# fnzhan/EMLight

Hardware: AMD Instinct MI355X
Metric: training images/sec (regression step: DenseNet-BC fwd + Sinkhorn loss + bwd + Adam) (higher is better)
Workload: dtype f32; 1 GPU; RegressionNetwork train step, BASELINE configs[1]; per_gpu_batch=64, global_batch=64, anchors=128, parallelism=single

## Files before the change

### emlight_amd/RegressionNetwork/dense_engine_bwd.py

```python
import ctypes
import os

import torch

from .. import _lib
from .._knobs import knob_choice, knob_flag


def _r16(v):
    return (v + 15) // 16 * 16


def _side_stream(dev, prio):
    if prio <= 0:
        return torch.cuda.Stream(device=dev, priority=prio)
    hip = ctypes.CDLL("libamdhip64.so")
    h = ctypes.c_void_p()
    with torch.cuda.device(dev):
        rc = hip.hipStreamCreateWithPriority(ctypes.byref(h), ctypes.c_uint(1), ctypes.c_int(prio))
    if rc != 0:
        raise RuntimeError("hipStreamCreateWithPriority failed (%d)" % rc)
    return torch.cuda.ExternalStream(h.value, device=dev)


# ... 15 lines not shown
class _BwdBuffers:
    def gf12(self, r):
        if self.GF12[r] is None:
            self.GF12[r] = self._gf12_new()
        return self.GF12[r]

    def __init__(self, enc, ws, dev):
        f32 = dict(dtype=torch.float32, device=dev)
        self.G = [torch.zeros(blk["P"], blk["ld"], **f32) for blk in ws.blocks]
        self.GF = torch.zeros(ws.F.shape[0], ws.F.shape[1], **f32)
        maxP = ws.blocks[0]["P"]
        self.DZ = torch.empty(2, maxP, 48, **f32)
        self.ring = max(1, int(os.environ.get("EML_WGRAD_RING", 4))) if enc.overlap_wgrad(dev) else 1
        self.GF12 = [None] * self.ring
        self._gf12_new = lambda: torch.empty(maxP, 12, **f32)
        self.N12 = torch.empty(maxP, 12, **f32)
        self.TOP = torch.empty(2 * maxP * 12, **f32) if knob_flag("EML_DGRAD_TOP", True) else None
        kp, ko, g = enc.kp_max, max(enc.ko_max, 48), enc.grid_max
        self.Wd = [[torch.empty(lay["Kp"] * 48, **f32) for lay in blk["layers"]] for blk in ws.blocks]
        self.WdT = [torch.empty(blk["trans"]["Kp"] * blk["trans"]["Ko"], **f32) for blk in ws.blocks]
        self.permutes = None
        self.coef = torch.zeros(8, max(kp, ko), **f32)
        self.part2 = torch.zeros(2, g * kp * 2, dtype=torch.float64, device=dev)
        self.partW = torch.empty(g * max(kp * 48, 2 * 27 * 256, 4 * 1024), **f32)
        i32 = dict(dtype=torch.int32, device=dev)
        self.cond = [[torch.zeros(lay["Kp"], **i32) for lay in blk["layers"]] for blk in ws.blocks]
        self.condT = [torch.zeros(blk["trans"]["Kp"], **i32) for blk in ws.blocks]
        self.any_ill = torch.zeros(1, **i32)
        self.dg_grid = 128
        self.dg_scratch = torch.empty(self.dg_grid * kp, dtype=torch.float64, device=dev)
        self.side = None
        if enc.overlap_wgrad(dev):
            m = int(os.environ.get("EML_CU_SPLIT", 0))
            self.main_masked = None
            if m > 1:
                n_cu = torch.cuda.get_device_properties(dev).multi_processor_count
                self.side = _masked_stream(dev, n_cu, lambda i: i % m == m - 1)
                self.main_masked = _masked_stream(dev, n_cu, lambda i: i % m != m - 1)
            else:
                self.side = _side_stream(dev, int(os.environ.get("EML_SIDE_PRIO", 0)))
            self.partW3 = [torch.empty(g * 2 * 27 * 256, **f32) for _ in range(self.ring)]
            self.ev_ready = [torch.cuda.Event() for _ in range(self.ring)]
            self.ev_done = [None] * self.ring


def run_backward(enc, ws, x, gpooled, need_x=False, need_params=None):
    if getattr(ws, "bwd", None) is None:
        ws.bwd = _BwdBuffers(enc, ws, x.device)
    masked = getattr(ws.bwd, "main_masked", None)
    if masked is None:
        return _run_backward(enc, ws, x, gpooled, need_x, need_params)
    cur = torch.cuda.current_stream(x.device)
    masked.wait_stream(cur)
# ... 85 lines not shown
                                                    blk["P"], st), "eml_dense_grad_materialize_f32")

    cf, k = enc.trans_cout[-1], enc.avgpool
    ldF = ws.F.shape[1]
    _lib.check(L.eml_dense_head_pool_bwd_f32(p(gpooled), p(ws.F), ldF, cf, B, ws.hf, ws.wf, k, p(bw.GF), ldF, st),
               "eml_dense_head_pool_bwd_f32")
    dY, ld_dy = bw.GF, ldF
    nb = len(ws.blocks)
    for bi in reversed(range(nb)):
        blk, tr = ws.blocks[bi], ws.blocks[bi]["trans"]
        mod = getattr(f, "denseblock%d" % (bi + 1))
        T, LN = getattr(f, "transition%d" % (bi + 1)), getattr(f, "last_norm%d" % (bi + 1))
        P, Hb, Wb, ld, ctot = blk["P"], blk["H"], blk["W"], blk["ld"], blk["Ctot"]
        cout, Ko, kpt = tr["Cout"], tr["Ko"], tr["Kp"]
        Pn = B * (Hb // 2) * (Wb // 2)
        Gbuf = bw.G[bi]
        gl0 = sum(enc.block_layers[:bi])
        top2 = bw.TOP[:2 * P * 12].view(2, P, 12) if bw.TOP is not None else None
        _lib.check(L.eml_dense_bn_bwd_stats_f32(p(dY), ld_dy, p(tr["T"]), Ko, None, 0, 0, cout, Pn, p(tr["tmean"]),
                                                p(tr["tistd"]), p(part), Gb, st), "eml_dense_bn_bwd_stats_f32")
        finalize(Gb, 2 * cout, Pn, LN, tr["tmean"], tr["tistd"], cout, Ko, coef=0)
        _lib.check(L.eml_dense_conv1x1_bwd_weight_f32(
            p(tr["A"]), kpt, Pn, Hb // 2, Wb // 2, 0, kpt, ctot, p(tr["one"]), p(tr["zero"]), p(dY), ld_dy, p(tr["T"]),
            Ko, p(cA), p(cB), p(cC), cout, p(bw.partW), gr(T.conv.weight), G, None, None, 0, None, 0, None, None, st),
            "eml_dense_conv1x1_bwd_weight_f32")
        _lib.check(L.eml_dense_conv1x1_bwd_data_f32(
            p(dY), ld_dy, p(tr["T"]), Ko, p(cA), p(cB), p(cC), Ko, p(bw.WdT[bi]), None, ld, p(tr["scale"]),
            p(tr["shift"]), None, None, Pn, Hb, Wb, 1, kpt, p(Gbuf), ld, 0, p(part), G, p(tr["mask16"]), st),
            "eml_dense_conv1x1_bwd_data_f32")
        finalize(G, 2 * kpt, P, T.norm, blk["mean"], blk["istd"], ctot, kpt, coef=None, s_acc=False, conv=T.conv,
                 cond=bw.condT[bi])
        dgamma_direct(blk, ld, P, Hb, Wb, 1, dY, ld_dy, tr["T"], Ko, coefs[0], cout, T.conv, ctot, tr["scale"], tr["shift"],
                      bw.condT[bi], T.norm)
        def conv2_backward(l, slot, n12=False, narrow_lo=None, top=False):
            lay = blk["layers"][l]
            Lm = getattr(mod, "denselayer%d" % (l + 1))
            cin, kp, z, dz = lay["Cin"], lay["Kp"], blk["Z"][l], bw.DZ[slot]
            gsrc = (p(bw.N12), 12, 0) if n12 else (p(top2[1]), 12, 0) if top else (p(Gbuf), ld, cin)
            r = ring[0] = (ring[0] + 1) % bw.ring
            if bw.side is not None and bw.ev_done[r] is not None:
                main.wait_event(bw.ev_done[r])
            fold = (bw.side is None and c3_fold
                    and L.eml_dense_conv3x3_bwd_fused_supported(gsrc[1], gsrc[2], ld, cin) == 1)
            q = ws.drop_plan[bi][l] if ws.drop_plan is not None else 0.0
            drop = (ws.drop_key, gl0 + l, q) if q > 0 else ()
            if fold:
                fn = "eml_dense_conv3x3_bwd_fused_drop_f32" if drop else "eml_dense_conv3x3_bwd_fused_f32"
# ... 40 lines not shown
                    parr([bw.part2[s_] for s_ in slots]), (ctypes.c_int * len(layers))(*[y["Kp"] for y in lays]),
                    P, k_hi, p(Gbuf), ld, Gd, parr([y["mask"] for y in lays]), p(top2), st),
                    "eml_dense_conv1x1_bwd_data_multi_top_f32")
                return
            _lib.check(L.eml_dense_conv1x1_bwd_data_multi_f32(
                len(layers), parr([bw.DZ[s_] for s_ in slots]), None, None, None, None,
                parr([bw.Wd[bi][l_] for l_ in layers]),
                parr([y["scale1"] for y in lays]), parr([y["shift1"] for y in lays]),
                parr([bw.part2[s_] for s_ in slots]), (ctypes.c_int * len(layers))(*[y["Kp"] for y in lays]),
                None, ld, None, None, P, k_lo, k_hi, p(Gbuf), ld, Gd,
                parr([y["mask"] for y in lays]), st),
                "eml_dense_conv1x1_bwd_data_multi_f32")

        def bn1_finalize(l, Lm, slot, c_lo, c_hi, rows=None):
            lay = blk["layers"][l]
            finalize(Gd if rows is None else rows, 2 * lay["Kp"], P, Lm.norm1, blk["mean"], blk["istd"], lay["Cin"], lay["Kp"], coef=None,
                     s_acc=True, src=bw.part2[slot], c_lo=c_lo, c_hi=c_hi, conv=Lm.conv1, cond=bw.cond[bi][l])

        def bn1_direct(l, Lm, slot):
            lay = blk["layers"][l]
            dgamma_direct(blk, ld, P, Hb, Wb, 0, bw.DZ[slot], 48, None, 0, None, 48, Lm.conv1, lay["Cin"], lay["scale1"],
                          lay["shift1"], bw.cond[bi][l], Lm.norm1)

        l = len(blk["layers"]) - 1
        have_top = False
        while l >= 0:
            if l >= 1:
                la, lb = l, l - 1
                cin_a, cin_b = blk["layers"][la]["Cin"], blk["layers"][lb]["Cin"]
                Lma = conv2_backward(la, 0, narrow_lo=cin_b, top=have_top)
                bn1_finalize(la, Lma, 0, cin_b, cin_a, rows=Gw)
                Lmb = conv2_backward(lb, 1, n12=True)
                to_top = (top2 is not None and lb >= 2 and blk["layers"][la]["mask"] is not None and bw.side is None
                          and cin_b >= 24 and cin_b % 4 == 0)
                dgrad([la, lb], [0, 1], 0, cin_b, top=to_top)
                have_top = to_top
                bn1_finalize(la, Lma, 0, 0, cin_b)
                bn1_finalize(lb, Lmb, 1, 0, blk["layers"][lb]["Kp"])
                bn1_direct(la, Lma, 0)
                bn1_direct(lb, Lmb, 1)
                l -= 2
            else:
                Lm0 = conv2_backward(l, 0)
                dgrad([l], [0], 0, blk["layers"][l]["Cin"])
                bn1_finalize(l, Lm0, 0, 0, blk["layers"][l]["Kp"])
                bn1_direct(l, Lm0, 0)
                l -= 1
        c0b = blk["C0"]
        norm0_fused = bi == 0 and knob_flag("EML_NORM0_FUSED", True) and c0b % 4 == 0 and c0b <= 32
        if not norm0_fused:
            materialize(Gbuf, blk, 0, c0b)
        dY, ld_dy = Gbuf, ld
    b0 = ws.blocks[0]
    c0 = enc.c_init
    if norm0_fused:
        _lib.check(L.eml_dense_norm0_bwd_stats_f32(p(dY), ld_dy, p(ws.Y0), c0, p(ws.scale0), p(ws.shift0), p(sB), p(sC), c0,
                                                   b0["P"], p(ws.mean0), p(ws.istd0), p(part), Gb, st),
                   "eml_dense_norm0_bwd_stats_f32")
    else:
        _lib.check(L.eml_dense_bn_bwd_stats_f32(p(dY), ld_dy, p(ws.Y0), c0, p(b0["X"]), b0["ld"], 1, c0, b0["P"],
                                                p(ws.mean0), p(ws.istd0), p(part), Gb, st), "eml_dense_bn_bwd_stats_f32")
    finalize(Gb, 2 * c0, b0["P"], f.norm0, ws.mean0, ws.istd0, c0, _r16(c0), coef=0)
    if norm0_fused:
# ... 18 lines not shown
```

### emlight_amd/_lib.py

```python
import ctypes
import os
import threading

_HERE = os.path.dirname(os.path.abspath(__file__))
LIB_PATH = os.environ.get("EML_LIB_PATH") or os.path.join(_HERE, "libemlight_hip.so")

_f32p = ctypes.c_void_p
_i32p = ctypes.c_void_p
_f64p = ctypes.c_void_p
_stream = ctypes.c_void_p
_int = ctypes.c_int
_u64 = ctypes.c_ulonglong

ABI_VERSION = 31

SIGNATURES = {
    "eml_abi_version": (_int, []),
    "eml_last_error": (ctypes.c_char_p, []),
    "eml_sg_rasterise_f32": (_int, [_f32p, _f32p, _f32p, _f32p, _int, _int, _int, _int, _stream]),
    "eml_sg_rasterise_ex_f32": (_int, [_f32p, _f32p, _f32p, _f32p, _int, _int, _int, _int, _int, ctypes.c_void_p, _stream]),
    "eml_sg_rasterise_bwd_colors_f32": (_int, [_f32p, _f32p, _f32p, _f32p, _int, _int, _int, _int, _stream]),
    "eml_emd_anchor_cost_f32": (_int, [_f32p, _f32p, _int, _stream]),
    "eml_sinkhorn_schedule_f32": (_int, [_f32p, _f32p, ctypes.c_long, ctypes.c_double, ctypes.c_double, _int,
                                         ctypes.c_double, _f32p, _f32p, _i32p, _f32p, _stream]),
# ... 135 lines not shown
    "eml_dense_dropout_mask_u16": (_int, [_u64, _int, ctypes.c_double, ctypes.c_long, ctypes.c_void_p, _stream]),
    "eml_dense_pool_act_f32": (_int, [_f32p, _int, _int, _int, _int, _int, _f32p, _f32p, _f32p, _int, ctypes.c_void_p,
                                      _stream]),
    "eml_dense_head_pool_fwd_f32": (_int, [_f32p, _int, _int, _int, _int, _int, _int, _f32p, _stream]),
    "eml_dense_conv3x3_bwd_data_f32": (_int, [_f32p, _int, _int, _f32p, _f32p, _f32p, _f32p, _f32p, _int, _int, _int,
                                              _f32p, _int, _f32p, _int, _int, _f32p, _f32p, _f32p, _stream]),
    "eml_dense_conv3x3_bwd_fused_supported": (_int, [_int, _int, _int, _int]),
    "eml_dense_conv3x3_bwd_fused_f32": (_int, [_f32p, _int, _int, _f32p, _f32p, _f32p, _f32p, _f32p, _int, _int, _int, _f64p, _int,
                                               _f32p, _int, _int, _f32p, _f32p, _f32p, _f32p, _f32p, _f32p, _f32p, _stream]),
    "eml_dense_conv3x3_bwd_data_drop_f32": (_int, [_f32p, _int, _int, _f32p, _f32p, _f32p, _f32p, _f32p, _int, _int, _int,
                                                   _f32p, _int, _f32p, _int, _int, _f32p, _f32p, _f32p, _u64, _int,
                                                   ctypes.c_double, _stream]),
    "eml_dense_conv3x3_bwd_fused_drop_f32": (_int, [_f32p, _int, _int, _f32p, _f32p, _f32p, _f32p, _f32p, _int, _int, _int,
                                                    _f64p, _int, _f32p, _int, _int, _f32p, _f32p, _f32p, _f32p, _f32p, _f32p,
                                                    _f32p, _u64, _int, ctypes.c_double, _stream]),
    "eml_dense_conv3x3_bwd_weight_f32": (_int, [_f32p, _int, _int, _f32p, _f32p, _f32p, _int, _int, _int, _f32p,
                                                _f32p, _int, _stream]),
    "eml_dense_bn_bwd_finalize_f32": (_int, [_f32p, _int, _int, ctypes.c_double, _f32p, _f32p, _f32p, _int, _int,
                                             _int, _f32p, _f32p, _f32p, _f32p, _f32p, _f32p, _f32p, _int, _int, _int,
                                             _f32p, _f32p, _f32p, _int, _i32p, _i32p, _stream]),
    "eml_dense_bn_dgamma_direct_f32": (_int, [_f32p, _int, ctypes.c_long, _int, _int, _int, _f32p, _int, _f32p, _int,
                                              _f32p, _f32p, _f32p, _int, _f32p, _int, _f32p, _f32p, _f32p, _f32p, _i32p,
                                              _f32p, _f32p, _int, _stream]),
    "eml_dense_conv1x1_bwd_weight_f32": (_int, [_f32p, _int, ctypes.c_long, _int, _int, _int, _int, _int, _f32p,
                                                _f32p, _f32p, _int, _f32p, _int, _f32p, _f32p, _f32p, _int, _f32p,
                                                _f32p, _int, _f32p, _f32p, _int, _f32p, _int, _f32p, _f32p, _stream]),
    "eml_dense_conv1x1_bwd_narrow_f32": (_int, [_f32p, _f32p, _int, _int, _f32p, _int, _f32p, _f32p, _f32p, _f32p,
                                                ctypes.c_long, _f32p, _int, _f32p, _f32p, _int, _int, _stream]),
    "eml_dense_permute_w1_bwd_f32": (_int, [_f32p, _int, _int, _int, _int, _f32p, _stream]),
    "eml_dense_conv1x1_bwd_data_f32": (_int, [_f32p, _int, _f32p, _int, _f32p, _f32p, _f32p, _int, _f32p, _f32p,
                                              _int, _f32p, _f32p, _f32p, _f32p, ctypes.c_long, _int, _int, _int,
                                              _int, _f32p, _int, _int, _f32p, _int, ctypes.c_void_p, _stream]),
    "eml_dense_conv1x1_bwd_data_multi_f32": (_int, [_int] + [ctypes.c_void_p] * 10 + [_f32p, _int, _f32p, _f32p,
                                                    ctypes.c_long, _int, _int, _f32p, _int, _int, ctypes.c_void_p,
                                                    _stream]),
    "eml_dense_conv1x1_bwd_data_multi_top_f32": (_int, [ctypes.c_void_p] * 6 + [ctypes.c_long, _int, _f32p, _int, _int,
                                                        ctypes.c_void_p, _f32p, _stream]),
    "eml_dense_grad_materialize_f32": (_int, [_f32p, _int, _f32p, _int, _f32p, _f32p, _int, _int, ctypes.c_long,
                                              _stream]),
    "eml_dense_bn_bwd_stats_f32": (_int, [_f32p, _int, _f32p, _int, _f32p, _int, _int, _int, ctypes.c_long, _f32p,
                                          _f32p, _f32p, _int, _stream]),
    "eml_dense_norm0_bwd_stats_f32": (_int, [_f32p, _int, _f32p, _int, _f32p, _f32p, _f32p, _f32p, _int, ctypes.c_long, _f32p, _f32p,
                                             ctypes.c_void_p, _int, _stream]),
    "eml_dense_conv0_bwd_weight_fused_f32": (_int, [_f32p, _f32p, _int, _f32p, _int, _f32p, _f32p, _f32p, _f32p, _f32p, _f32p, _f32p,
                                                    _int, _int, _int, _f32p, _f32p, _int, _stream]),
    "eml_dense_conv0_bwd_weight_f32": (_int, [_f32p, _f32p, _int, _f32p, _int, _f32p, _int, _f32p, _f32p, _f32p,
# ... 79 lines not shown
```

### emlight_amd/csrc/dense_bwd.hip

```cpp
#include "eml_common.h"
#include "eml_dropout.h"

#include <cstdint>
#include <cstdlib>
#include <type_traits>

namespace {

using f32x4 = __attribute__((ext_vector_type(4))) float;

__device__ __forceinline__ f32x4 mfma16(float a, float b, f32x4 c) {
  return __builtin_amdgcn_mfma_f32_16x16x4f32(a, b, c, 0, 0, 0);
}
__device__ __forceinline__ float f4c(const float4& v, int t) { return t == 0 ? v.x : t == 1 ? v.y : t == 2 ? v.z : v.w; }
__device__ __forceinline__ double shfl_xor_d(double v, int m) { return __shfl_xor(v, m, 64); }

constexpr int kTH = 8, kTW = 32, kHH = kTH + 2, kHW = kTW + 2;

constexpr int kPSG = 14;
constexpr int kBD = 512;
constexpr int kGRows = 2;
constexpr int kGPass = kHH / kGRows;

template <bool FUSE, bool WIDE, int TH, bool DROP = false>
// ... 1415 lines not shown
#pragma unroll
      for (int g = 0; g < 4; ++g) {
        const int ch = GW * cg + VEC * (4 * kk + g) + t;
        if (cg < ngroups && ch < Kp) {
#pragma unroll
          for (int n = 0; n < 3; ++n) out[(size_t)ch * 48 + 16 * n + r] = acc[i][t][n][g];
        }
      }
  }
  if constexpr (NARROW) {
    __syncthreads();
    double* red = reinterpret_cast<double*>(&dz_l[0][0]);
#pragma unroll
    for (int g = 0; g < 4; ++g) {
#pragma unroll
      for (int o = 1; o < 16; o <<= 1) ns1[g] += shfl_xor_d(ns1[g], o);
      if (r == 0 && kk < 3) red[wave * 12 + 4 * kk + g] = ns1[g];
    }
    __syncthreads();
    if (tid < 12) {
      double* dst = na.partials + ((size_t)blockIdx.x * Kp + na.k_lo + tid) * 2;
      dst[0] = (red[tid] + red[12 + tid]) + (red[24 + tid] + red[36 + tid]);
      dst[1] = 0.0;
    }
  }
}

template <bool POOL, bool RES , int NCH = 4>
__global__ __launch_bounds__(256) void conv1x1_bwd_data_kernel(
    const float* __restrict__ DY, int ld_dy, const float* __restrict__ Zr, int ld_z, const float* __restrict__ cA,
    const float* __restrict__ cB, const float* __restrict__ cC, int Ko, const float* __restrict__ Wd,
    const float* __restrict__ X, int ldx, const float* __restrict__ scale1, const float* __restrict__ shift1,
    const float* __restrict__ mean, const float* __restrict__ istd, int P, int Hin, int Win, int Kp,
    float* __restrict__ Gd, int ldg, int accumulate, double* __restrict__ partials ) {
  extern __shared__ __attribute__((aligned(16))) float smem[];
  double* sacc = reinterpret_cast<double*>(smem);
  const int tid = threadIdx.x, lane = tid & 63, wave = tid >> 6;
  const int r = lane & 15, kk = lane >> 4;
  for (int e = tid; e < 4 * Kp * 2; e += 256) sacc[e] = 0.0;
  __syncthreads();
  double* my = sacc + (size_t)wave * Kp * 2;
  const int nnt = Kp >> 4, njo = Ko >> 4;
  const int ntiles = (P + 255) >> 8;
  const int Wo = Win >> 1, Ho = Hin >> 1;

  for (int tile = blockIdx.x; tile < ntiles; tile += gridDim.x) {
// ... 1118 lines not shown
}

__global__ __launch_bounds__(256) void head_pool_bwd_kernel(const float* __restrict__ gp, const float* __restrict__ F,
                                                            int ldf, int C, int B, int H, int W, int k,
                                                            float* __restrict__ dF, int ldd) {
  const int Ho = H / k, Wo = W / k;
  const size_t total = (size_t)B * H * W * C;
  const float inv = 1.0f / (float)(k * k);
  for (size_t e = (size_t)blockIdx.x * 256 + threadIdx.x; e < total; e += (size_t)gridDim.x * 256) {
    const int c = (int)(e % C);
    const size_t p = e / C;
    const int xx = (int)(p % W);
    const size_t rest = p / W;
    const int yy = (int)(rest % H), b = (int)(rest / H);
    const int oy = yy / k, ox = xx / k;
    float v = 0.f;
    if (oy < Ho && ox < Wo && F[p * ldf + c] > 0.f) v = gp[(((size_t)b * C + c) * Ho + oy) * Wo + ox] * inv;
    dF[p * ldd + c] = v;
  }
}

}

__global__ __launch_bounds__(256) void bn_dgamma_direct_partial_kernel(
    const float* __restrict__ X, int ldx, long P, int Hin, int Win, int pool, const float* __restrict__ DY, int ld_dy,
    const float* __restrict__ Zr, int ld_z, const float* __restrict__ cA, const float* __restrict__ cB,
    const float* __restrict__ cC, int Cout, const float* __restrict__ W, int Cin, const float* __restrict__ scale1,
    const float* __restrict__ shift1, const float* __restrict__ mean, const float* __restrict__ istd,
    const int* __restrict__ cond, double* __restrict__ partial) {
  __shared__ int list[384];
  __shared__ int cnt;
  __shared__ float wcol[192], co[3][192];
  __shared__ double red[4];
  const int tid = threadIdx.x;
  if (tid == 0) cnt = 0;
  __syncthreads();
  for (int c = tid; c < Cin; c += 256)
    if (cond[c]) list[atomicAdd(&cnt, 1)] = c;
  __syncthreads();
  const int n = cnt;
  if (n == 0) return;
  for (int o = tid; o < Cout; o += 256) {
    co[0][o] = Zr ? cA[o] : 1.f;
    co[1][o] = Zr ? cB[o] : 0.f;
    co[2][o] = Zr ? cC[o] : 0.f;
  }
  const long per = (P + gridDim.x - 1) / gridDim.x, p_lo = (long)blockIdx.x * per, p_hi = min(P, p_lo + per);
  const int Ho = Hin >> 1, Wo = Win >> 1;
  for (int li = 0; li < n; ++li) {
    const int c = list[li];
    __syncthreads();
    for (int o = tid; o < Cout; o += 256) wcol[o] = W[(size_t)o * Cin + c];
    __syncthreads();
    const float s1 = scale1[c], t1 = shift1[c];
    const double mu = mean[c], is = istd[c];
    double acc = 0.0;
    for (long p = p_lo + tid; p < p_hi; p += 256) {
      const float x = X[(size_t)p * ldx + c];
      if (fmaf(x, s1, t1) > 0.f) {
        long pp = p;
        if (pool) {
          const long b = p / ((long)Hin * Win), rem = p - b * (long)Hin * Win;
          const int y = (int)(rem / Win), xx = (int)(rem - (long)y * Win);
          pp = (b * Ho + (y >> 1)) * Wo + (xx >> 1);
        }
        const float* dy = DY + (size_t)pp * ld_dy;
        const float* zr = Zr ? Zr + (size_t)pp * ld_z : dy;
        double d = 0.0;
        for (int o = 0; o < Cout; ++o) d += (double)wcol[o] * (double)fmaf(co[0][o], dy[o], fmaf(co[1][o], zr[o], co[2][o]));
        if (pool) d *= 0.25;
        acc += d * (((double)x - mu) * is);
      }
    }
#pragma unroll
    for (int o = 32; o > 0; o >>= 1) acc += shfl_xor_d(acc, o);
    if ((tid & 63) == 0) red[tid >> 6] = acc;
    __syncthreads();
    if (tid == 0) partial[(size_t)blockIdx.x * Cin + c] = (red[0] + red[1]) + (red[2] + red[3]);
  }
}

__global__ __launch_bounds__(256) void bn_dgamma_direct_reduce_kernel(const double* __restrict__ partial, int R, int Cin,
                                                                      const int* __restrict__ cond,
                                                                      float* __restrict__ dgamma) {
  const int c = blockIdx.x * 256 + threadIdx.x;
  if (c >= Cin || !cond[c]) return;
  double s = 0.0;
  for (int g = 0; g < R; ++g) s += partial[(size_t)g * Cin + c];
  dgamma[c] = (float)s;
}

extern "C" int eml_dense_conv3x3_bwd_data_f32(const float* G, int ldg, int c0, const float* W2, const float* Z,
                                              const float* zmean, const float* zistd, float* DZ, int B, int H, int W,
                                              double* partials, int grid, const float* X, int ldx, int cx,
                                              const float* sB, const float* sC, float* GF, eml_stream_t stream) {
  if (!G || !W2 || !Z || !zmean || !zistd || !DZ || !partials || B < 1 || H < 1 || W < 1 || grid < 1 || (c0 & 1) ||
      (ldg & 1))
    return eml::fail(EML_EINVAL, "eml_dense_conv3x3_bwd_data_f32: bad arguments");
  if (X) {
    if (!sB || !sC || !GF || (ldx & 1))
      return eml::fail(EML_EINVAL, "eml_dense_conv3x3_bwd_data_f32: fused affine needs X, sB, sC, GF");
    if (cx < 0 || (cx & 1)) return eml::fail(EML_EINVAL, "eml_dense_conv3x3_bwd_data_f32: cx must be even");
  }
  static const bool narrow = [] { const char* v = getenv("EML_D3_NARROW"); return v && v[0] == '1'; }();
  static const bool tall = [] { const char* v = getenv("EML_D3_SHORT"); return !(v && v[0] == '1'); }();
  const auto al16 = [](const void* q) { return (reinterpret_cast<uintptr_t>(q) & 15) == 0; };
  const bool wide = !narrow && (ldg & 3) == 0 && (c0 & 3) == 0 && al16(G) &&
                    (!X || ((ldx & 3) == 0 && (cx & 3) == 0 && al16(X) && al16(sB) && al16(sC) && al16(GF)));
#define EML_LAUNCH_D3(FUSEV, WIDEV, THV)                                                                                \
  hipLaunchKernelGGL((conv3x3_bwd_data_kernel<FUSEV, WIDEV, THV>), dim3(grid), dim3(THV * 64), 0, (hipStream_t)stream, G, ldg, \
                     c0, W2, Z, zmean, zistd, DZ, B, H, W, partials, X, ldx, cx, sB, sC, GF, eml::DropKey{})
  if (X) {
// ... 219 lines not shown
                     R, pstride, count, gamma, mean, istd, C, Cpad, training, dgamma, dbeta, cA, cB, cC, sB, sC,
                     s_accumulate, c_lo, c_hi, beta, W, dW, w_rows, W ? cond : nullptr, W ? any_cond : nullptr);
  return eml::check_launch("eml_dense_bn_bwd_finalize_f32");
}

extern "C" int eml_dense_bn_dgamma_direct_f32(const float* X, int ldx, long P, int Hin, int Win, int pool, const float* DY,
                                              int ld_dy, const float* Zr, int ld_z, const float* cA, const float* cB,
                                              const float* cC, int Cout, const float* W, int Cin, const float* scale1,
                                              const float* shift1, const float* mean, const float* istd, const int* cond,
                                              double* scratch, float* dgamma, int grid, eml_stream_t stream) {
  if (!X || !DY || !W || !scale1 || !shift1 || !mean || !istd || !cond || !scratch || !dgamma || P < 1 || grid < 1 ||
      Cin < 1 || Cin > 384 || Cout < 1 || Cout > 192 || Cin > ldx || Cout > ld_dy || (Zr && (!cA || !cB || !cC || Cout > ld_z)) ||
      (pool && ((Hin | Win) & 1)))
    return eml::fail(EML_EINVAL, "eml_dense_bn_dgamma_direct_f32: bad arguments (Cin <= 384, Cout <= 192, even maps when pooled)");
  hipLaunchKernelGGL(bn_dgamma_direct_partial_kernel, dim3(grid), dim3(256), 0, (hipStream_t)stream, X, ldx, P, Hin, Win,
                     pool, DY, ld_dy, Zr, ld_z, cA, cB, cC, Cout, W, Cin, scale1, shift1, mean, istd, cond, scratch);
  int rc = eml::check_launch("eml_dense_bn_dgamma_direct_f32(partial)");
  if (rc) return rc;
  hipLaunchKernelGGL(bn_dgamma_direct_reduce_kernel, dim3((Cin + 255) / 256), dim3(256), 0, (hipStream_t)stream, scratch,
                     grid, Cin, cond, dgamma);
  return eml::check_launch("eml_dense_bn_dgamma_direct_f32(reduce)");
}

extern "C" int eml_dense_conv1x1_bwd_weight_f32(const float* X, int ldx, long P, int Hin, int Win, int pool, int Kp,
                                                int Cin, const float* scale1, const float* shift1, const float* DY,
                                                int ld_dy, const float* Zr, int ld_z, const float* cA, const float* cB,
                                                const float* cC, int Cout, float* partial, float* dW, int grid,
                                                float* dz_out, const float* W1, int k_lo, const float* G, int ldg,
                                                float* N12, double* partials_n, eml_stream_t stream) {
  if (dz_out && (Cout != 48 || pool))
    return eml::fail(EML_EINVAL, "eml_dense_conv1x1_bwd_weight_f32: dz_out is for dense layers (Cout == 48, no pool)");
  if (N12 && (Cout != 48 || pool || !W1 || !G || !partials_n || k_lo < 0 || (k_lo & 1) || k_lo + 12 > Cin || (ldg & 1) ||
              (ldg != 12 && k_lo + 12 > ldg)))
    return eml::fail(EML_EINVAL, "eml_dense_conv1x1_bwd_weight_f32: fused narrow pass needs a dense layer, W1, G, partials_n "
                                 "and an even k_lo with k_lo + 12 <= Cin (k_lo=%d, Cin=%d)", k_lo, Cin);
  if (!X || !scale1 || !shift1 || !DY || !Zr || !cA || !cB || !cC || !partial || !dW || P < 1 || grid < 1 || Kp < 32 ||
      (Kp & 15) || Cin > Kp || Cout < 1)
    return eml::fail(EML_EINVAL, "eml_dense_conv1x1_bwd_weight_f32: bad arguments");
  const int nchunks = (Cout + 47) / 48;
  for (int ch = 0; ch < nchunks; ++ch) {
    const int n0 = ch * 48, nv = (Cout - n0 < 48) ? Cout - n0 : 48;
    int n_load = ((ld_dy < ld_z ? ld_dy : ld_z) - n0) & ~3;
    if (n_load > 48) n_load = 48;
    if (n_load < nv) return eml::fail(EML_EINVAL, "eml_dense_conv1x1_bwd_weight_f32: DY/Zr rows narrower than Cout");
    const NarrowArgs na{W1, G, N12, partials_n, Cin, k_lo, ldg};
    static const int vec_env = [] { const char* v = getenv("EML_W1_VEC"); return v ? atoi(v) : 0; }();
    const bool vec4 = !pool && (ldx & 3) == 0 && (reinterpret_cast<uintptr_t>(X) & 15) == 0 &&
                      vec_env == 4;
    if (vec4 && N12 && vec_env == 4)
      hipLaunchKernelGGL((conv1x1_bwd_weight_kernel<false, true, 4>), dim3(grid), dim3(256), 0, (hipStream_t)stream, X, ldx,
                         (int)P, Hin, Win, Kp, scale1, shift1, DY + n0, ld_dy, Zr + n0, ld_z, cA + n0, cB + n0, cC + n0,
                         nv, n_load, partial, dz_out, na);
    else if (vec4 && !N12)
      hipLaunchKernelGGL((conv1x1_bwd_weight_kernel<false, false, 4>), dim3(grid), dim3(256), 0, (hipStream_t)stream, X, ldx,
                         (int)P, Hin, Win, Kp, scale1, shift1, DY + n0, ld_dy, Zr + n0, ld_z, cA + n0, cB + n0, cC + n0,
                         nv, n_load, partial, dz_out, na);
    else if (pool)
      hipLaunchKernelGGL((conv1x1_bwd_weight_kernel<true, false>), dim3(grid), dim3(256), 0, (hipStream_t)stream, X, ldx,
                         (int)P, Hin, Win, Kp, scale1, shift1, DY + n0, ld_dy, Zr + n0, ld_z, cA + n0, cB + n0, cC + n0,
                         nv, n_load, partial, nullptr, na);
    else if (N12)
      hipLaunchKernelGGL((conv1x1_bwd_weight_kernel<false, true>), dim3(grid), dim3(256), 0, (hipStream_t)stream, X, ldx,
                         (int)P, Hin, Win, Kp, scale1, shift1, DY + n0, ld_dy, Zr + n0, ld_z, cA + n0, cB + n0, cC + n0,
// ... 283 lines not shown
```

### include/emlight_hip.h

```cpp
#ifndef EMLIGHT_HIP_H
#define EMLIGHT_HIP_H

#include <stddef.h>
#include <stdint.h>

#ifdef __cplusplus
extern "C" {
#endif

typedef void* eml_stream_t;

#define EML_OK 0
#define EML_EINVAL (-1)
#define EML_ELAUNCH (-2)

#define EML_MAX_EPS 64

#define EML_ABI_VERSION 31
int eml_abi_version(void);
const char* eml_last_error(void);

int eml_sg_rasterise_f32(const float* dirs, const float* sizes, const float* colors,
                         float* out, int B, int N, int H, int W, eml_stream_t stream);

// ... 142 lines not shown
                                         double* partials, int grid, const float* X, int ldx, int cx,
                                         const float* sB, const float* sC, float* GF, const float* scale2,
                                         const float* shift2, float* partialW, float* dW2, unsigned long long seed,
                                         int layer, double p, eml_stream_t stream);

int eml_dense_conv3x3_bwd_weight_f32(const float* G, int ldg, int c0, const float* Z,
                                     const float* scale2, const float* shift2, int B, int H, int W,
                                     float* partial, float* dW2, int grid, eml_stream_t stream);

int eml_dense_bn_bwd_finalize_f32(const double* partials, int R, int pstride, double count,
                                  const float* gamma, const float* mean, const float* istd, int C,
                                  int Cpad, int training, float* dgamma, float* dbeta, float* cA,
                                  float* cB, float* cC, float* sB, float* sC, int s_accumulate,
                                  int c_lo, int c_hi, const float* beta, const float* W, const float* dW,
                                  int w_rows, int* cond, int* any_cond, eml_stream_t stream);

int eml_dense_bn_dgamma_direct_f32(const float* X, int ldx, long P, int Hin, int Win, int pool,
                                   const float* DY, int ld_dy, const float* Zr, int ld_z, const float* cA,
                                   const float* cB, const float* cC, int Cout, const float* W, int Cin,
                                   const float* scale1, const float* shift1, const float* mean,
                                   const float* istd, const int* cond, double* scratch, float* dgamma,
                                   int grid, eml_stream_t stream);

int eml_dense_conv1x1_bwd_weight_f32(const float* X, int ldx, long P, int Hin, int Win, int pool,
                                     int Kp, int Cin, const float* scale1, const float* shift1,
                                     const float* DY, int ld_dy, const float* Zr, int ld_z,
                                     const float* cA, const float* cB, const float* cC, int Cout,
                                     float* partial, float* dW, int grid, float* dz_out,
                                     const float* W1, int k_lo, const float* G, int ldg, float* N12,
                                     double* partials_n, eml_stream_t stream);

int eml_dense_permute_w1_bwd_f32(const float* W, int Cout, int Cin, int Kp, int Ko, float* Wd,
                                 eml_stream_t stream);

int eml_dense_conv1x1_bwd_data_f32(const float* DY, int ld_dy, const float* Zr, int ld_z,
                                   const float* cA, const float* cB, const float* cC, int Ko,
                                   const float* Wd, const float* X, int ldx, const float* scale1,
                                   const float* shift1, const float* mean, const float* istd, long P,
                                   int Hin, int Win, int pool, int Kp, float* G, int ldg,
                                   int accumulate, double* partials, int grid,
                                   const unsigned short* relu_mask16, eml_stream_t stream);

int eml_dense_conv1x1_bwd_data_multi_f32(int n_layers, const float* const* DZ, const float* const* Zr,
                                         const float* const* cA, const float* const* cB,
                                         const float* const* cC, const float* const* Wd,
                                         const float* const* scale1, const float* const* shift1,
// ... 205 lines not shown
```

Before: 567.9 images/s.

## Fuse paired BN dgamma-direct launches and add multi-chunk transition weight-gradient kernel

New measurement: 567.7 images/s. Within noise of the previous version (-0.0%).

```diff
diff --git a/emlight_amd/RegressionNetwork/dense_engine_bwd.py b/emlight_amd/RegressionNetwork/dense_engine_bwd.py
--- a/emlight_amd/RegressionNetwork/dense_engine_bwd.py
+++ b/emlight_amd/RegressionNetwork/dense_engine_bwd.py
@@ -61,13 +61,19 @@
         self.permutes = None
         self.coef = torch.zeros(8, max(kp, ko), **f32)
         self.part2 = torch.zeros(2, g * kp * 2, dtype=torch.float64, device=dev)
-        self.partW = torch.empty(g * max(kp * 48, 2 * 27 * 256, 4 * 1024), **f32)
+        L = _lib.lib()
+        self.wchunks = [L.eml_dense_conv1x1_bwd_weight_chunks_per_pass(blk["trans"]["Kp"], blk["trans"]["Cout"], 0)
+                        for blk in ws.blocks]
+        kp_t = max(max(n, 1) * blk["trans"]["Kp"] for n, blk in zip(self.wchunks, ws.blocks))
+        self.partW = torch.empty(g * max(kp * 48, kp_t * 48, 2 * 27 * 256, 4 * 1024), **f32)
         i32 = dict(dtype=torch.int32, device=dev)
         self.cond = [[torch.zeros(lay["Kp"], **i32) for lay in blk["layers"]] for blk in ws.blocks]
         self.condT = [torch.zeros(blk["trans"]["Kp"], **i32) for blk in ws.blocks]
         self.any_ill = torch.zeros(1, **i32)
         self.dg_grid = 128
         self.dg_scratch = torch.empty(self.dg_grid * kp, dtype=torch.float64, device=dev)
+        n_pair = L.eml_dense_bn_dgamma_direct_pair_scratch_doubles(self.dg_grid, kp, kp)
+        self.dg_pair = torch.zeros(n_pair, dtype=torch.float64, device=dev) if n_pair else None
         self.side = None
         if enc.overlap_wgrad(dev):
             m = int(os.environ.get("EML_CU_SPLIT", 0))
@@ -199,7 +205,7 @@
         finalize(Gb, 2 * cout, Pn, LN, tr["tmean"], tr["tistd"], cout, Ko, coef=0)
         _lib.check(L.eml_dense_conv1x1_bwd_weight_f32(
             p(tr["A"]), kpt, Pn, Hb // 2, Wb // 2, 0, kpt, ctot, p(tr["one"]), p(tr["zero"]), p(dY), ld_dy, p(tr["T"]),
-            Ko, p(cA), p(cB), p(cC), cout, p(bw.partW), gr(T.conv.weight), G, None, None, 0, None, 0, None, None, st),
+            Ko, p(cA), p(cB), p(cC), cout, p(bw.partW), gr(T.conv.weight), G, None, None, 0, None, bw.wchunks[bi], None, None, st),
             "eml_dense_conv1x1_bwd_weight_f32")
         _lib.check(L.eml_dense_conv1x1_bwd_data_f32(
             p(dY), ld_dy, p(tr["T"]), Ko, p(cA), p(cB), p(cC), Ko, p(bw.WdT[bi]), None, ld, p(tr["scale"]),
@@ -286,6 +292,17 @@
             dgamma_direct(blk, ld, P, Hb, Wb, 0, bw.DZ[slot], 48, None, 0, None, 48, Lm.conv1, lay["Cin"], lay["scale1"],
                           lay["shift1"], bw.cond[bi][l], Lm.norm1)
 
+        def bn1_direct_pair(la, Lma, lb, Lmb):
+            if not direct:
+                return
+            ya, yb = blk["layers"][la], blk["layers"][lb]
+            _lib.check(L.eml_dense_bn_dgamma_direct_pair_f32(
+                p(blk["X"]), ld, P, p(blk["mean"]), p(blk["istd"]),
+                p(bw.DZ[0]), p(Lma.conv1.weight), ya["Cin"], p(ya["scale1"]), p(ya["shift1"]), p(bw.cond[bi][la]),
+                gr(Lma.norm1.weight), ya["Kp"],
+                p(bw.DZ[1]), p(Lmb.conv1.weight), yb["Cin"], p(yb["scale1"]), p(yb["shift1"]), p(bw.cond[bi][lb]),
+                gr(Lmb.norm1.weight), yb["Kp"], p(bw.dg_pair), bw.dg_grid, st), "eml_dense_bn_dgamma_direct_pair_f32")
+
         l = len(blk["layers"]) - 1
         have_top = False
         while l >= 0:
@@ -301,8 +318,11 @@
                 have_top = to_top
                 bn1_finalize(la, Lma, 0, 0, cin_b)
                 bn1_finalize(lb, Lmb, 1, 0, blk["layers"][lb]["Kp"])
-                bn1_direct(la, Lma, 0)
-                bn1_direct(lb, Lmb, 1)
+                if bw.dg_pair is not None:
+                    bn1_direct_pair(la, Lma, lb, Lmb)
+                else:
+                    bn1_direct(la, Lma, 0)
+                    bn1_direct(lb, Lmb, 1)
                 l -= 2
             else:
                 Lm0 = conv2_backward(l, 0)
diff --git a/emlight_amd/_lib.py b/emlight_amd/_lib.py
--- a/emlight_amd/_lib.py
+++ b/emlight_amd/_lib.py
@@ -181,6 +181,12 @@
     "eml_dense_bn_dgamma_direct_f32": (_int, [_f32p, _int, ctypes.c_long, _int, _int, _int, _f32p, _int, _f32p, _int,
                                               _f32p, _f32p, _f32p, _int, _f32p, _int, _f32p, _f32p, _f32p, _f32p, _i32p,
                                               _f32p, _f32p, _int, _stream]),
+    "eml_dense_bn_dgamma_direct_pair_scratch_doubles": (ctypes.c_size_t, [_int, _int, _int]),
+    "eml_dense_bn_dgamma_direct_pair_f32": (_int, [_f32p, _int, ctypes.c_long, _f32p, _f32p,
+                                                   _f32p, _f32p, _int, _f32p, _f32p, _i32p, _f32p, _int,
+                                                   _f32p, _f32p, _int, _f32p, _f32p, _i32p, _f32p, _int,
+                                                   _f64p, _int, _stream]),
+    "eml_dense_conv1x1_bwd_weight_chunks_per_pass": (_int, [_int, _int, _int]),
     "eml_dense_conv1x1_bwd_weight_f32": (_int, [_f32p, _int, ctypes.c_long, _int, _int, _int, _int, _int, _f32p,
                                                 _f32p, _f32p, _int, _f32p, _int, _f32p, _f32p, _f32p, _int, _f32p,
                                                 _f32p, _int, _f32p, _f32p, _int, _f32p, _int, _f32p, _f32p, _stream]),
diff --git a/emlight_amd/csrc/dense_bwd.hip b/emlight_amd/csrc/dense_bwd.hip
--- a/emlight_amd/csrc/dense_bwd.hip
+++ b/emlight_amd/csrc/dense_bwd.hip
@@ -1461,6 +1461,192 @@
       double* dst = na.partials + ((size_t)blockIdx.x * Kp + na.k_lo + tid) * 2;
       dst[0] = (red[tid] + red[12 + tid]) + (red[24 + tid] + red[36 + tid]);
       dst[1] = 0.0;
+    }
+  }
+}
+
+template <int NC, int NTL>
+__global__ __launch_bounds__(256, 1) void conv1x1_bwd_weight_chunks_kernel(
+    const float* __restrict__ X, int ldx, int P, int Kp, const float* __restrict__ scale1,
+    const float* __restrict__ shift1, const float* __restrict__ DY, int ld_dy, const float* __restrict__ Zr, int ld_z,
+    const float* __restrict__ cA, const float* __restrict__ cB, const float* __restrict__ cC,
+    int n_valid ,
+    int n_load ,
+    float* __restrict__ partial ) {
+  static_assert(NC >= 2 && NC <= 3 && NTL >= 1 && NTL <= (NC == 3 ? 1 : 3), "2 chunks, or 3 with one tile in the last");
+  __shared__ __attribute__((aligned(16))) float dz_l[NC][2][64 * 48];
+  __shared__ __attribute__((aligned(16))) float co_l[NC][3 * 48];
+  const int tid = threadIdx.x, lane = tid & 63, wave = tid >> 6;
+  const int r = lane & 15, kk = lane >> 4;
+  constexpr int MAXG = 3;
+  const int ngroups = (Kp + 31) / 32;
+  float sv[MAXG][2], tv[MAXG][2];
+  int coff[MAXG];
+#pragma unroll
+  for (int i = 0; i < MAXG; ++i) {
+    const int cg = wave + 4 * i;
+    const int ch = 32 * cg + 2 * r;
+    const bool gv = cg < ngroups && ch < Kp;
+    coff[i] = gv ? ch : 0;
+#pragma unroll
+    for (int t = 0; t < 2; ++t) {
+      sv[i][t] = gv ? scale1[ch + t] : 0.f;
+      tv[i][t] = gv ? shift1[ch + t] : 0.f;
+    }
+  }
+  const int spix = tid >> 2, sq = tid & 3;
+  if (tid < 48 * NC) {
+    const int c = tid / 48, o = tid - 48 * c;
+    const bool v = tid < n_valid;
+    co_l[c][o] = v ? cA[tid] : 0.f;
+    co_l[c][48 + o] = v ? cB[tid] : 0.f;
+    co_l[c][96 + o] = v ? cC[tid] : 0.f;
+  }
+  __syncthreads();
+  f32x4 acc[NC][MAXG][2][3];
+#pragma unroll
+  for (int c = 0; c < NC; ++c)
+#pragma unroll
+    for (int i = 0; i < MAXG; ++i)
+#pragma unroll
+      for (int t = 0; t < 2; ++t)
+#pragma unroll
+        for (int n = 0; n < 3; ++n) acc[c][i][t][n] = f32x4{0.f, 0.f, 0.f, 0.f};
+
+  const int nchunks = (P + 63) >> 6;
+  const int ngw = (ngroups > wave) ? (ngroups - wave + 3) >> 2 : 0;
+
+  float4 rdy[NC][3], rzr[NC][3];
+  bool rpv = false;
+  auto stage_load = [&](int chunk) {
+    const int p = chunk * 64 + spix;
+    rpv = chunk < nchunks && p < P;
+    const size_t pc = rpv ? p : 0;
+#pragma unroll
+    for (int c = 0; c < NC; ++c)
+#pragma unroll
+      for (int j = 0; j < (c == NC - 1 ? NTL : 3); ++j) {
+        const int col = 48 * c + 4 * (sq + 4 * j);
+        const bool cv = col < n_load;
+        rdy[c][j] = cv ? *reinterpret_cast<const float4*>(DY + pc * ld_dy + col) : make_float4(0.f, 0.f, 0.f, 0.f);
+        rzr[c][j] = cv ? *reinterpret_cast<const float4*>(Zr + pc * ld_z + col) : make_float4(0.f, 0.f, 0.f, 0.f);
+      }
+  };
+  auto stage_write = [&](int buf) {
+#pragma unroll
+    for (int c = 0; c < NC; ++c)
+#pragma unroll
+      for (int j = 0; j < (c == NC - 1 ? NTL : 3); ++j) {
+        const int col = 4 * (sq + 4 * j);
+        const float4 sa = *reinterpret_cast<const float4*>(co_l[c] + col);
+        const float4 sb = *reinterpret_cast<const float4*>(co_l[c] + 48 + col);
+        const float4 sc = *reinterpret_cast<const float4*>(co_l[c] + 96 + col);
+        float4 v;
+        v.x = rpv ? fmaf(sa.x, rdy[c][j].x, fmaf(sb.x, rzr[c][j].x, sc.x)) : 0.f;
+        v.y = rpv ? fmaf(sa.y, rdy[c][j].y, fmaf(sb.y, rzr[c][j].y, sc.y)) : 0.f;
+        v.z = rpv ? fmaf(sa.z, rdy[c][j].z, fmaf(sb.z, rzr[c][j].z, sc.z)) : 0.f;
+        v.w = rpv ? fmaf(sa.w, rdy[c][j].w, fmaf(sb.w, rzr[c][j].w, sc.w)) : 0.f;
+        *reinterpret_cast<float4*>(dz_l[c][buf] + spix * 48 + col) = v;
+      }
+  };
+  auto chunk_loop = [&](auto ngw_c) {
+    constexpr int NGW = decltype(ngw_c)::value;
+    constexpr int UQ = 4, NBUF = 2, NB = 16 / UQ, AHEAD = NBUF - 1;
+    float2 xr[NBUF][UQ][NGW > 0 ? NGW : 1];
+    auto load_batch = [&](int chunk, int q0, float2 (&dst)[UQ][NGW > 0 ? NGW : 1]) {
+#pragma unroll
+      for (int u = 0; u < UQ; ++u) {
+        const int pc = min(chunk * 64 + 4 * (q0 + u) + kk, P - 1);
+        const float* xp = X + (size_t)pc * ldx;
+#pragma unroll
+        for (int i = 0; i < NGW; ++i) dst[u][i] = *reinterpret_cast<const float2*>(xp + coff[i]);
+      }
+    };
+    stage_load(blockIdx.x);
+    stage_write(0);
+    if constexpr (NGW > 0) {
+#pragma unroll
+      for (int a = 0; a < AHEAD; ++a) load_batch(min((int)blockIdx.x, nchunks - 1), a * UQ, xr[a]);
+    }
+    __syncthreads();
+    int it = 0;
+    for (int chunk = blockIdx.x; chunk < nchunks; chunk += gridDim.x, ++it) {
+      const int buf = it & 1;
+      stage_load(chunk + gridDim.x);
+      if constexpr (NGW > 0) {
+        float bzq[2][NC][3];
+#pragma unroll
+        for (int c = 0; c < NC; ++c)
+#pragma unroll
+          for (int n = 0; n < (c == NC - 1 ? NTL : 3); ++n) bzq[0][c][n] = dz_l[c][buf][kk * 48 + 16 * n + r];
+#pragma unroll
+        for (int bi = 0; bi < NB; ++bi) {
+          const int q0 = bi * UQ;
+          if (bi + AHEAD < NB)
+            load_batch(chunk, q0 + AHEAD * UQ, xr[(bi + AHEAD) % NBUF]);
+          else
+            load_batch(min(chunk + (int)gridDim.x, nchunks - 1), (bi + AHEAD - NB) * UQ, xr[(bi + AHEAD) % NBUF]);
+          __builtin_amdgcn_sched_barrier(0);
+#pragma unroll
+          for (int u = 0; u < UQ; ++u) {
+            const int pl = 4 * (q0 + u) + kk;
+            const bool pvu = chunk * 64 + pl < P;
+            float bz[NC][3];
+#pragma unroll
+            for (int c = 0; c < NC; ++c)
+#pragma unroll
+              for (int n = 0; n < (c == NC - 1 ? NTL : 3); ++n) bz[c][n] = bzq[(q0 + u) & 1][c][n];
+            if (q0 + u + 1 < 16) {
+#pragma unroll
+              for (int c = 0; c < NC; ++c)
+#pragma unroll
+                for (int n = 0; n < (c == NC - 1 ? NTL : 3); ++n)
+                  bzq[(q0 + u + 1) & 1][c][n] = dz_l[c][buf][(pl + 4) * 48 + 16 * n + r];
+            }
+#pragma unroll
+            for (int i = 0; i < NGW; ++i) {
+              const float2 xv = xr[bi % NBUF][u][i];
+              float av[2];
+              av[0] = 0.f + fmaxf(fmaf(xv.x, sv[i][0], tv[i][0]), 0.f);
+              av[1] = 0.f + fmaxf(fmaf(xv.y, sv[i][1], tv[i][1]), 0.f);
+              if (!pvu) av[0] = av[1] = 0.f;
+#pragma unroll
+              for (int c = 0; c < NC; ++c)
+#pragma unroll
+                for (int n = 0; n < (c == NC - 1 ? NTL : 3); ++n)
+#pragma unroll
+                  for (int t = 0; t < 2; ++t) acc[c][i][t][n] = mfma16(av[t], bz[c][n], acc[c][i][t][n]);
+            }
+          }
+          __builtin_amdgcn_sched_barrier(0);
+        }
+      }
+      stage_write(buf ^ 1);
+      eml::lds_barrier();
+    }
+  };
+  switch (ngw) {
+    case 0: chunk_loop(std::integral_constant<int, 0>{}); break;
+    case 1: chunk_loop(std::integral_constant<int, 1>{}); break;
+    case 2: chunk_loop(std::integral_constant<int, 2>{}); break;
+    default: chunk_loop(std::integral_constant<int, MAXG>{}); break;
+  }
+#pragma unroll
+  for (int c = 0; c < NC; ++c) {
+    float* out = partial + ((size_t)c * gridDim.x + blockIdx.x) * Kp * 48;
+#pragma unroll
+    for (int i = 0; i < MAXG; ++i) {
+      const int cg = wave + 4 * i;
+#pragma unroll
+      for (int t = 0; t < 2; ++t)
+#pragma unroll
+        for (int g = 0; g < 4; ++g) {
+          const int ch = 32 * cg + 2 * (4 * kk + g) + t;
+          if (cg < ngroups && ch < Kp) {
+#pragma unroll
+            for (int n = 0; n < (c == NC - 1 ? NTL : 3); ++n) out[(size_t)ch * 48 + 16 * n + r] = acc[c][i][t][n][g];
+          }
+        }
     }
   }
 }
@@ -2625,7 +2811,7 @@
 
 }
 
-__global__ __launch_bounds__(256) void bn_dgamma_direct_partial_kernel(
+__device__ __forceinline__ bool bn_dgamma_direct_partial(
     const float* __restrict__ X, int ldx, long P, int Hin, int Win, int pool, const float* __restrict__ DY, int ld_dy,
     const float* __restrict__ Zr, int ld_z, const float* __restrict__ cA, const float* __restrict__ cB,
     const float* __restrict__ cC, int Cout, const float* __restrict__ W, int Cin, const float* __restrict__ scale1,
@@ -2642,7 +2828,7 @@
     if (cond[c]) list[atomicAdd(&cnt, 1)] = c;
   __syncthreads();
   const int n = cnt;
-  if (n == 0) return;
+  if (n == 0) return false;
   for (int o = tid; o < Cout; o += 256) {
     co[0][o] = Zr ? cA[o] : 1.f;
     co[1][o] = Zr ? cB[o] : 0.f;
@@ -2681,6 +2867,17 @@
     __syncthreads();
     if (tid == 0) partial[(size_t)blockIdx.x * Cin + c] = (red[0] + red[1]) + (red[2] + red[3]);
   }
+  return true;
+}
+
+__global__ __launch_bounds__(256) void bn_dgamma_direct_partial_kernel(
+    const float* __restrict__ X, int ldx, long P, int Hin, int Win, int pool, const float* __restrict__ DY, int ld_dy,
+    const float* __restrict__ Zr, int ld_z, const float* __restrict__ cA, const float* __restrict__ cB,
+    const float* __restrict__ cC, int Cout, const float* __restrict__ W, int Cin, const float* __restrict__ scale1,
+    const float* __restrict__ shift1, const float* __restrict__ mean, const float* __restrict__ istd,
+    const int* __restrict__ cond, double* __restrict__ partial) {
+  bn_dgamma_direct_partial(X, ldx, P, Hin, Win, pool, DY, ld_dy, Zr, ld_z, cA, cB, cC, Cout, W, Cin, scale1, shift1, mean, istd,
+                           cond, partial);
 }
 
 __global__ __launch_bounds__(256) void bn_dgamma_direct_reduce_kernel(const double* __restrict__ partial, int R, int Cin,
@@ -2691,6 +2888,52 @@
   double s = 0.0;
   for (int g = 0; g < R; ++g) s += partial[(size_t)g * Cin + c];
   dgamma[c] = (float)s;
+}
+
+struct DgammaPairLayer {
+  const float* DY;
+  const float* W;
+  const float* scale1;
+  const float* shift1;
+  const int* cond;
+  float* dgamma;
+  int Cin;
+};
+__global__ __launch_bounds__(256) void bn_dgamma_direct_pair_kernel(const float* __restrict__ X, int ldx, long P,
+                                                                    const float* __restrict__ mean,
+                                                                    const float* __restrict__ istd, DgammaPairLayer la,
+                                                                    DgammaPairLayer lb, double* __restrict__ part_a,
+                                                                    double* __restrict__ part_b, unsigned* ticket) {
+  __shared__ bool last;
+  const bool fa = bn_dgamma_direct_partial(X, ldx, P, 0, 0, 0, la.DY, 48, nullptr, 0, nullptr, nullptr, nullptr, 48, la.W, la.Cin,
+                                           la.scale1, la.shift1, mean, istd, la.cond, part_a);
+  __syncthreads();
+  const bool fb = bn_dgamma_direct_partial(X, ldx, P, 0, 0, 0, lb.DY, 48, nullptr, 0, nullptr, nullptr, nullptr, 48, lb.W, lb.Cin,
+                                           lb.scale1, lb.shift1, mean, istd, lb.cond, part_b);
+  if (!fa && !fb) return;
+  __syncthreads();
+  if (threadIdx.x == 0) {
+    __threadfence();
+    const unsigned t = atomicAdd(ticket, 1u);
+    last = t == gridDim.x - 1;
+    if (last) __threadfence();
+  }
+  __syncthreads();
+  if (!last) return;
+  const int R = gridDim.x;
+  for (int half = 0; half < 2; ++half) {
+    const DgammaPairLayer& L = half ? lb : la;
+    const double* part = half ? part_b : part_a;
+    if (!(half ? fb : fa)) continue;
+    for (int c = threadIdx.x; c < L.Cin; c += 256) {
+      if (!L.cond[c]) continue;
+      double s = 0.0;
+      for (int g = 0; g < R; ++g)
+        s += __hip_atomic_load(part + (size_t)g * L.Cin + c, __ATOMIC_RELAXED, __HIP_MEMORY_SCOPE_AGENT);
+      L.dgamma[c] = (float)s;
+    }
+  }
+  if (threadIdx.x == 0) *ticket = 0u;
 }
 
 extern "C" int eml_dense_conv3x3_bwd_data_f32(const float* G, int ldg, int c0, const float* W2, const float* Z,
@@ -2956,6 +3199,38 @@
   return eml::check_launch("eml_dense_bn_dgamma_direct_f32(reduce)");
 }
 
+extern "C" size_t eml_dense_bn_dgamma_direct_pair_scratch_doubles(int grid, int Kp_a, int Kp_b) {
+  static const bool on = [] { const char* v = getenv("EML_DGAMMA_PAIR"); return !(v && v[0] == '0'); }();
+  if (!on || grid < 1 || Kp_a < 1 || Kp_b < 1 || Kp_a > 384 || Kp_b > 384) return 0;
+  return (size_t)grid * ((size_t)Kp_a + Kp_b) + 1;
+}
+
+extern "C" int eml_dense_bn_dgamma_direct_pair_f32(const float* X, int ldx, long P, const float* mean, const float* istd,
+                                                   const float* DZ_a, const float* W_a, int Cin_a, const float* scale1_a,
+                                                   const float* shift1_a, const int* cond_a, float* dgamma_a, int Kp_a,
+                                                   const float* DZ_b, const float* W_b, int Cin_b, const float* scale1_b,
+                                                   const float* shift1_b, const int* cond_b, float* dgamma_b, int Kp_b,
+                                                   double* scratch, int grid, eml_stream_t stream) {
+  if (!X || !mean || !istd || !DZ_a || !W_a || !scale1_a || !shift1_a || !cond_a || !dgamma_a || !DZ_b || !W_b || !scale1_b ||
+      !shift1_b || !cond_b || !dgamma_b || !scratch || P < 1 || grid < 1 || Cin_a < 1 || Cin_b < 1 || Cin_a > Kp_a ||
+      Cin_b > Kp_b || Kp_a > 384 || Kp_b > 384 || Cin_a > ldx || Cin_b > ldx)
+    return eml::fail(EML_EINVAL, "eml_dense_bn_dgamma_direct_pair_f32: bad arguments (Cin <= Kp <= 384, Cin <= ldx)");
+  double* part_a = scratch + 1, *part_b = part_a + (size_t)grid * Kp_a;
+  const DgammaPairLayer la{DZ_a, W_a, scale1_a, shift1_a, cond_a, dgamma_a, Cin_a};
+  const DgammaPairLayer lb{DZ_b, W_b, scale1_b, shift1_b, cond_b, dgamma_b, Cin_b};
+  hipLaunchKernelGGL(bn_dgamma_direct_pair_kernel, dim3(grid), dim3(256), 0, (hipStream_t)stream, X, ldx, P, mean, istd, la,
+                     lb, part_a, part_b, reinterpret_cast<unsigned*>(scratch));
+  return eml::check_launch("eml_dense_bn_dgamma_direct_pair_f32");
+}
+
+static bool wgrad_three_chunks_fit(int Cout) { return Cout > 96 && Cout <= 112; }
+
+extern "C" int eml_dense_conv1x1_bwd_weight_chunks_per_pass(int Kp, int Cout, int pool) {
+  static const int most = [] { const char* v = getenv("EML_TRANS_WGRAD_ONEPASS"); return !v || v[0] == '0' ? 0 : v[0] == '3' ? 3 : 2; }();
+  if (!most || pool || Cout <= 48 || Kp < 32 || Kp > 384) return 0;
+  return most == 3 && wgrad_three_chunks_fit(Cout) ? 3 : 2;
+}
+
 extern "C" int eml_dense_conv1x1_bwd_weight_f32(const float* X, int ldx, long P, int Hin, int Win, int pool, int Kp,
                                                 int Cin, const float* scale1, const float* shift1, const float* DY,
                                                 int ld_dy, const float* Zr, int ld_z, const float* cA, const float* cB,
@@ -2972,7 +3247,39 @@
       (Kp & 15) || Cin > Kp || Cout < 1)
     return eml::fail(EML_EINVAL, "eml_dense_conv1x1_bwd_weight_f32: bad arguments");
   const int nchunks = (Cout + 47) / 48;
+  int cap = (!N12 && !dz_out && !pool && Kp <= 384 && nchunks > 1) ? (ldg > 3 ? 3 : ldg) : 1;
+  if (cap == 3 && !wgrad_three_chunks_fit(Cout)) cap = 2;
+  const int ndisp = cap >= 2 ? (nchunks + cap - 1) / cap : nchunks;
+  const int per = cap >= 2 ? (nchunks + ndisp - 1) / ndisp : 1;
   for (int ch = 0; ch < nchunks; ++ch) {
+    const int nc = nchunks - ch < per ? nchunks - ch : per;
+    if (nc >= 2) {
+      const int n0 = ch * 48, nv = (Cout - n0 < 48 * nc) ? Cout - n0 : 48 * nc;
+      const int n_load = ((ld_dy < ld_z ? ld_dy : ld_z) - n0) & ~3;
+      if (n_load < nv) return eml::fail(EML_EINVAL, "eml_dense_conv1x1_bwd_weight_f32: DY/Zr rows narrower than Cout");
+      const int ntl = (nv - 48 * (nc - 1) + 15) / 16;
+      auto launch = [&](auto k) {
+        hipLaunchKernelGGL(k, dim3(grid), dim3(256), 0, (hipStream_t)stream, X, ldx, (int)P, Kp, scale1, shift1, DY + n0,
+                           ld_dy, Zr + n0, ld_z, cA + n0, cB + n0, cC + n0, nv, n_load, partial);
+      };
+      switch (nc * 4 + ntl) {
+        case 2 * 4 + 1: launch(conv1x1_bwd_weight_chunks_kernel<2, 1>); break;
+        case 2 * 4 + 2: launch(conv1x1_bwd_weight_chunks_kernel<2, 2>); break;
+        case 2 * 4 + 3: launch(conv1x1_bwd_weight_chunks_kernel<2, 3>); break;
+        default: launch(conv1x1_bwd_weight_chunks_kernel<3, 1>); break;
+      }
+      int rc = eml::check_launch("eml_dense_conv1x1_bwd_weight_f32(chunks)");
+      if (rc) return rc;
+      for (int c = 0; c < nc; ++c) {
+        const int nvc = (nv - 48 * c < 48) ? nv - 48 * c : 48;
+        hipLaunchKernelGGL(reduce_rows_kernel, dim3((Cin * 48 + 63) / 64), dim3(256), 0, (hipStream_t)stream,
+                           partial + (size_t)c * grid * Kp * 48, grid, (size_t)Kp * 48, 0, Cin, nvc, n0 + 48 * c, dW);
+        rc = eml::check_launch("eml_dense_conv1x1_bwd_weight_f32(reduce)");
+        if (rc) return rc;
+      }
+      ch += nc - 1;
+      continue;
+    }
     const int n0 = ch * 48, nv = (Cout - n0 < 48) ? Cout - n0 : 48;
     int n_load = ((ld_dy < ld_z ? ld_dy : ld_z) - n0) & ~3;
     if (n_load > 48) n_load = 48;
diff --git a/include/emlight_hip.h b/include/emlight_hip.h
--- a/include/emlight_hip.h
+++ b/include/emlight_hip.h
@@ -188,6 +188,15 @@
                                    const float* istd, const int* cond, double* scratch, float* dgamma,
                                    int grid, eml_stream_t stream);
 
+size_t eml_dense_bn_dgamma_direct_pair_scratch_doubles(int grid, int Kp_a, int Kp_b);
+int eml_dense_bn_dgamma_direct_pair_f32(const float* X, int ldx, long P, const float* mean, const float* istd,
+                                        const float* DZ_a, const float* W_a, int Cin_a, const float* scale1_a,
+                                        const float* shift1_a, const int* cond_a, float* dgamma_a, int Kp_a,
+                                        const float* DZ_b, const float* W_b, int Cin_b, const float* scale1_b,
+                                        const float* shift1_b, const int* cond_b, float* dgamma_b, int Kp_b,
+                                        double* scratch, int grid, eml_stream_t stream);
+
+int eml_dense_conv1x1_bwd_weight_chunks_per_pass(int Kp, int Cout, int pool);
 int eml_dense_conv1x1_bwd_weight_f32(const float* X, int ldx, long P, int Hin, int Win, int pool,
                                      int Kp, int Cin, const float* scale1, const float* shift1,
                                      const float* DY, int ld_dy, const float* Zr, int ld_z,
```
